# gregorgebhardt/gym-kilobots

Hardware: AMD Instinct MI355X
Metric: kilobot-steps/sec (higher is better)
Workload: dtype f32

## Files before the change

gym_kilobots_amd/csrc/kb_step_kernel.h:

```cpp
#pragma once
#include <type_traits>
#include <utility>

#include "kb_common.h"
#include "kb_objects.h"

namespace kb {

template <int DRIVE_MODE, int LIGHT_TYPE, bool OBJ, int FN = 0, int TIER = 0, bool POLY = true, bool SENSE = true, bool SLEEP = false>
__global__ void __launch_bounds__(TIER == 1 ? 64 : 64 * KB_MAX_WAVES, (TIER == 1 || TIER == 3) ? 2 : ((TIER == 2 || (FN != 0 && !OBJ)) ? KB_COMPACT_WAVES_PER_SIMD : KB_MIN_WAVES_PER_SIMD)) kb_step_kernel(const Params p) {
    constexpr bool WIDE = TIER == 1 || TIER == 3;
    constexpr bool BINS = !OBJ;
    constexpr int KRX = BINS ? KB_KREG_BINS : KREG;
    constexpr bool PAR_DS = FN != 0 && BINS;
    static_assert(!SLEEP || FN == 0 || !OBJ, "the fixed-size instantiations with objects do not carry the sleep state");
    extern __shared__ __align__(16) unsigned char smem[];
    constexpr bool SCOPED = KB_ARGS_SCOPED && FN != 0 && !OBJ;
    using ArgPtr = std::conditional_t<SCOPED, const __attribute__((address_space(4))) Params *, const Params *>;
    ArgPtr ka;
    if constexpr (SCOPED) ka = (ArgPtr)__builtin_amdgcn_kernarg_segment_ptr();
    else ka = &p;
#define KB_REARG() do { if constexpr (SCOPED) { ka = (ArgPtr)__builtin_amdgcn_kernarg_segment_ptr(); asm volatile("" : "+s"(ka)); } } while (0)
    {
        static_assert(sizeof(Params) >= 6 * 64, "the six lines asked for are kernel arguments");
// ... 310 lines not shown
                    float n = sqrtf(lgx * lgx + lgy * lgy);
                    float mx = lgx, my = lgy;
                    if (n > 0.01f) { mx = lgx / n * 0.01f; my = lgy / n * 0.01f; }
                    bvx = mx * WORLD_SCALE; bvy = my * WORLD_SCALE; bww = 0.0f;
                } break;
                default: break;
                }
            }
            if (ka->buf.cmd_vx) { ka->buf.cmd_vx[o + b] = bvx; ka->buf.cmd_vy[o + b] = bvy; ka->buf.cmd_w[o + b] = bww; }
            if (SLEEP) {
                if (drive && slp[q] < 0.0f && (bww * bww > 0.0f || bvx * bvx + bvy * bvy > 0.0f)) slp[q] = 0.0f;
                if (slp[q] < 0.0f) { bvx = 0.0f; bvy = 0.0f; bww = 0.0f; }
                active[b] = 0;
            }
            const float kl = (KB_LAW(q) == KB_DRIVE_SIMPLE_PHOTOTAXIS) ? 1.0f / (1.0f + h * 0.0f) : ka->kl_bot;
            bw[q] = bww * ka->ka_bot;
            int cx = (int)floorf((bx - ka->xmin) * ka->inv_cell);
            int cy = (int)floorf((by - ka->ymin) * ka->inv_cell);
            cx = cx < 0 ? 0 : (cx >= ka->gw ? ka->gw - 1 : cx);
            cy = cy < 0 ? 0 : (cy >= ka->gh ? ka->gh - 1 : cy);
            const int cell = cy * ka->gw + cx;
            if (BINS) {
                sbx[q] = bx; sby[q] = by; svx[q] = bvx * kl; svy[q] = bvy * kl; scell[q] = cx | (cy << 12);
                const int bi = (hashed ? (cell & ka->hmask) : cell) + 1;
                const unsigned old = atomicAdd(reinterpret_cast<unsigned *>(E1) + (bi >> 1), 1u << (16 * (bi & 1)));
                sarr[q] = (int)((old >> (16 * (bi & 1))) & 0xFFFFu);
                if (SENSE && ka->sense_s > 0) reinterpret_cast<unsigned short *>(lAcc)[b] = 0;
            } else {
                vel[b].x = bvx * kl; vel[b].y = bvy * kl;
                parent[b] = b;
                cellOf[b] = (unsigned short)cell;
                nextb[b] = (unsigned short)kb_exch16(head, hix(cell), (unsigned)b);
                if (SENSE && ka->sense_s > 0) newOff[b] = 0;
            }
        }
        if (tid < M) { start[N + tid].x = pos[N + tid].x; start[N + tid].y = pos[N + tid].y; objA0[tid] = objA[tid]; }
        if (tid < M) {
            vel[N + tid].x *= ka->kl_obj; vel[N + tid].y *= ka->kl_obj; objW[tid] *= ka->ka_obj;
            parent[N + tid] = N + tid;
            objCnt[tid] = 0;
            if (SLEEP) active[N + tid] = 0;
        }
        if (OBJ && tid >= M && tid < F) objCnt[tid] = 0;
        if (tid < M_COUNT && tid != M_STATUS) misc[tid] = 0;
        if (SLEEP && tid < 32) misc[M_WAKE + tid] = 0;
        KB_STAMP_PRE(16);
        __syncthreads();
        KB_STAMP(0);
        KB_RETID();
        KB_ABLATE_EXIT(1);
        auto ws_find = [&](int owner, unsigned key16) __attribute__((always_inline)) -> float {
            const int cnt = wsCnt[owner], off = wsOff[owner];
            if (oldInLds) {
                for (int s = 0; s < cnt; ++s)
                    if (oldKey[off + s] == (unsigned short)key16) {
                        const float a_ = oldAcc[off + s];
                        if (SLEEP) oldAcc[off + s] = -1.0f - a_;
                        return a_;
                    }
            } else {
                const unsigned key32 = key16 >= (unsigned)WALL_CODE ? KEY_WALL + (key16 - WALL_CODE)
                                     : (key16 >= (unsigned)OBJ_CODE ? KEY_OBJ + (key16 - OBJ_CODE) : key16);
                for (int s0 = 0; s0 < cnt; s0 += 4) {
                    unsigned k4[4];
#pragma unroll
                    for (int u = 0; u < 4; ++u) {
                        const int idx = off + s0 + u;
                        k4[u] = (s0 + u < cnt && idx < ka->cap) ? ka->buf.ws_key[wo + idx] : 0xFFFFFFFFu;
                    }
#pragma unroll
                    for (int u = 0; u < 4; ++u)
                        if (k4[u] == key32) {
                            const float a_ = ka->buf.ws_acc[wo + off + s0 + u];
                            if (SLEEP) ka->buf.ws_acc[wo + off + s0 + u] = -1.0f - a_;
                            return a_;
                        }
                }
            }
            return -1.0f;
        };
        bool big = false;
        int stageCap = 0, ncon = 0;
        unsigned newTotal = 0;
        if constexpr (BINS) {
            int gw_ = ka->gw, gh_ = ka->gh;
            float invCell_ = ka->inv_cell;
#define KB_GRID_ARGS() do { KB_REARG(); gw_ = ka->gw; gh_ = ka->gh; invCell_ = ka->inv_cell; } while (0)
            {
                const int nchunks = ldsb::bin_entries(ka->nhead) >> 3;
                if (nchunks <= nt) block_scan_bins<true>(E1, nchunks, 1, wsum, tid);
                else block_scan_bins<false>(E1, nchunks, (nchunks + nt - 1) / nt, wsum, tid);
            }
            KB_STAMP_PRE(31);
#pragma unroll
            for (int q = 0; q < BPT; ++q) {
                const int b = tid + q * nt;
                if (b >= N) continue;
                const int cell = SC_CY(scell[q]) * gw_ + SC_CX(scell[q]);
                const int bin = hashed ? (cell & ka->hmask) : cell;
                tmpSort[(int)E1[bin] + sarr[q]] = (unsigned short)b;
            }
            __syncthreads();
            KB_STAMP_PRE(32);
            KB_RETID();
#pragma unroll
            for (int q = 0; q < BPT; ++q) {
                const int b = tid + q * nt;
                if (b >= N) continue;
                const int cell = SC_CY(scell[q]) * gw_ + SC_CX(scell[q]);
                const int bin = hashed ? (cell & ka->hmask) : cell;
                const int s0 = (int)E1[bin], s1 = (int)E1[bin + 1];
                int rank = 0;
                if (s1 - s0 > 1)
                    for (int s_ = s0; s_ < s1; ++s_) rank += ((int)tmpSort[s_] < b) ? 1 : 0;
                const int sl = s0 + rank;
                ms[q] = sl;
                idOf[sl] = (unsigned short)b;
                if (hashed) cellOfSlot[sl] = (unsigned short)cell;
                pos[sl] = make_float2(sbx[q], sby[q]);
                vel[sl] = make_float2(svx[q], svy[q]);
                parent[sl] = (unsigned)sl;
            }
            if (tid < 4) {
                float z_ = 0.0f;
                asm volatile("" : "+v"(z_));
                vel[NB - 5 + tid] = make_float2(z_, z_);
            }
            KB_STAMP_PRE(33);
            KB_GRID_ARGS();
            __syncthreads();
            KB_STAMP(0);
            KB_RETID();
            KB_ABLATE_EXIT(2);
            if (SENSE && ka->sense_s > 0 && drive) {
#pragma unroll 1
                for (int q = 0; q < BPT; ++q) {
                    const int b = tid + q * nt;
                    if (b >= N) continue;
                    const int sl = q == 0 ? ms[0] : ms[BPT - 1];
                    const int sc = q == 0 ? scell[0] : scell[BPT - 1];
                    if (hashed) kb_sense_bins_hashed(pos, E1, cellOfSlot, reinterpret_cast<unsigned *>(lAcc), sl, SC_CX(sc), SC_CY(sc), gw_, gh_, ka->sense_s, ka->sense_r2, ka->hmask);
                    else kb_sense_bins(pos, E1, reinterpret_cast<unsigned *>(lAcc), sl, SC_CX(sc), SC_CY(sc), gw_, gh_, ka->sense_s, ka->sense_r2);
                }
            }
            constexpr int NR = FN ? 3 : 5;
            auto candidate_runs = [&](int sa, int cx, int cy, int (&lo)[NR], int (&hi)[NR], int (&sp)[NR], int (&tc)[5]) __attribute__((always_inline)) {
                const int gw = gw_, gh = gh_;
                const int cell = cy * gw + cx;
                const bool e_ok = cx + 1 < gw, n_ok = cy + 1 < gh, w_ok = cx > 0;
                tc[0] = cell; tc[1] = cell + 1; tc[2] = cell + gw; tc[3] = cell + gw + 1; tc[4] = cell + gw - 1;
                if constexpr (NR == 3) {
                    const int up = cell + gw;
                    const int e1 = (int)E1[cell + 1], e2 = (int)E1[e_ok ? cell + 2 : cell + 1];
                    const int u0 = (int)E1[n_ok ? (w_ok ? up - 1 : up) : 0], u1 = (int)E1[n_ok ? up : 0];
                    const int u2 = (int)E1[n_ok ? up + 1 : 0], u3 = (int)E1[n_ok ? (e_ok ? up + 2 : up + 1) : 0];
                    lo[0] = sa + 1; sp[0] = e1; hi[0] = e2;
                    lo[1] = u1; sp[1] = u2; hi[1] = u3;
                    lo[2] = u0; sp[2] = u1; hi[2] = u1;
                } else {
                    const bool ok[5] = {true, e_ok, n_ok, n_ok && e_ok, n_ok && w_ok};
#pragma unroll
                    for (int k = 0; k < 5; ++k) {
                        const int bin = hashed ? (tc[k] & ka->hmask) : tc[k];
                        const int l_ = ok[k] ? (int)E1[bin] : 0, h_ = ok[k] ? (int)E1[bin + 1] : 0;
                        lo[k] = k == 0 ? sa + 1 : l_; hi[k] = h_; sp[k] = h_;
                    }
// ... 33 lines not shown
                        const float dx = cp[u].x - pa.x, dy = cp[u].y - pa.y;
                        const float dd = dx * dx + dy * dy;
                        bool hit = base + u < tot && !(dd > rr2);
                        if (hashed) {
                            int want = tc[0];
#pragma unroll
                            for (int k = 1; k < 5; ++k) if (ck[u] == k) want = tc[k];
                            hit = hit && cc[u] == want;
                        }
                        if (hit) cb(cs[u], ck[u]);
                    }
                }
            };
            unsigned pl0[BPT], pl1[BPT];
            unsigned snb[BPT], snm[BPT];
#pragma unroll
            for (int q = 0; q < BPT; ++q) {
                const int b = tid + q * nt;
                pl0[q] = 0u; pl1[q] = 0u; snb[q] = 0u; snm[q] = 0u;
                if (b >= N) continue;
                const int sa = ms[q];
                unsigned cnt = 0, nbb = 0, l0 = 0u, l1 = 0u;
                for_partners(sa, SC_CX(scell[q]), SC_CY(scell[q]), [&](int sl, int k) __attribute__((always_inline)) {
                    const unsigned e16 = (unsigned)sl | ((unsigned)k << 12);
                    const unsigned sh = e16 << (16u * (nbb & 1u));
                    l0 |= nbb < 2u ? sh : 0u;
                    l1 |= (nbb >= 2u && nbb < 4u) ? sh : 0u;
                    nbb++;
                    if (((cnt >> (6 * k)) & 63u) == 63u) atomicOr(&misc[M_STATUS], 4u);
                    else cnt += 1u << (6 * k);
                });
                pl0[q] = l0; pl1[q] = l1; snb[q] = nbb;
                unsigned wm = 0u;
                const float ax = pos[sa].x, ay = pos[sa].y;
#pragma unroll
                for (int wl = 0; wl < 4; ++wl) {
                    float dist, nx, ny;
                    wall_geom(*ka, wl, ax, ay, dist, nx, ny);
                    if (dist * dist > rw2) continue;
                    wm |= (1u << wl) | (dist < 0.0f ? 16u << wl : 0u);
                }
                scell[q] |= (int)(wm << 24);
                unsigned mine = nbb + (unsigned)__popc(wm & 15u);
                dirCnt[sa] = cnt;
                if (mine > (unsigned)S) { atomicOr(&misc[M_STATUS], 2u); atomicAdd(&misc[M_XTRA], mine - (unsigned)S); mine = S; }
                wsCntNew[b] = (unsigned char)mine;
                snm[q] = mine;
            }
            KB_STAMP_PRE(17);
            unsigned myOff[BPT];
            {
                static_assert(BPT == 2 && MAX_WAVES <= 8, "two rows of per-wave sums in the 16-word scratch");
                const unsigned inc0 = wave_incl_scan(snm[0]), inc1 = wave_incl_scan(snm[1]);
                if (lane == 63) { wsum[wave] = inc0; wsum[8 + wave] = inc1; }
                KB_GRID_ARGS();
                __syncthreads();
                KB_ABLATE_EXIT(3);
                unsigned b0 = 0, b1 = 0, t0 = 0, t1 = 0;
                for (int w = 0; w < nw; ++w) {
                    const unsigned s0 = wsum[w], s1 = wsum[8 + w];
                    if (w < wave) { b0 += s0; b1 += s1; }
                    t0 += s0; t1 += s1;
                }
                myOff[0] = b0 + inc0 - snm[0]; myOff[1] = t0 + b1 + inc1 - snm[1];
                newTotal = t0 + t1;
            }
            KB_STAMP(1);
            KB_RETID();
            KB_ABLATE_EXIT(4);
            if (SENSE && ka->sense_s > 0 && drive) {
#pragma unroll
                for (int q = 0; q < BPT; ++q) {
                    const int b = tid + q * nt;
                    if (b < N) ka->buf.nbr_count[o + b] = (unsigned)reinterpret_cast<unsigned short *>(lAcc)[ms[q]];
                }
                __syncthreads();
            }
            const unsigned extras = misc[M_XTRA];
            const int capS = FN ? capL_ : min(capL_, ka->cap);
            big = ka->solver_mode >= 3 || newTotal + extras > (unsigned)capS;
            stageCap = big ? ka->cap : capS;
            if (newTotal + extras > (unsigned)stageCap && tid == 0) atomicOr(&misc[M_STATUS], 1u);
            ncon = (int)min(newTotal + extras, (unsigned)stageCap);
            auto stage_pass = [&](unsigned *sPair, unsigned *sInfo) __attribute__((always_inline)) {
#pragma unroll
            for (int q = 0; q < BPT; ++q) {
                const int b = tid + q * nt;
                if (b >= N) continue;
                const int sa = ms[q], cx = SC_CX(scell[q]), cy = SC_CY(scell[q]);
                const unsigned nbb = snb[q];
                const unsigned wm = (unsigned)scell[q] >> 24;
                const unsigned ntot = nbb + (unsigned)__popc(wm & 15u);
                newOff[b] = (unsigned short)myOff[q];
                if (ntot == 0u) continue;
                const unsigned base = myOff[q], nst = snm[q];
                const int cell = cy * gw_ + cx;
                const unsigned common = ((unsigned)(cx & 1) << 12) | ((unsigned)(cy & 1) << 13) | (sa > (int)E1[hashed ? (cell & ka->hmask) : cell] ? 1u << 14 : 0u);
                int curk = -1;
                unsigned jk = 0;
                unsigned wleft = wm & 15u;
                for (unsigned j = 0; j < ntot; ++j) {
                    unsigned pr, inf;
                    if (j < nbb) {
                        unsigned e16;
                        if (j < 4u) e16 = ((j < 2u ? pl0[q] : pl1[q]) >> (16u * (j & 1u))) & 0xFFFFu;
                        else {
                            unsigned idx = 0, f16 = 0;
                            for_partners(sa, cx, cy, [&](int sl, int kk) __attribute__((always_inline)) { if (idx == j) f16 = (unsigned)sl | ((unsigned)kk << 12); idx++; });
                            e16 = f16;
                        }
                        const int k = (int)(e16 >> 12);
                        if (k != curk) { curk = k; jk = 0; } else jk++;
                        if (jk > 255u) { jk = 255u; atomicOr(&misc[M_STATUS], 4u); }
                        pr = (unsigned)sa | ((e16 & 0xFFFu) << 16);
                        inf = (unsigned)k | (jk << 4) | common;
                    } else {
                        const int wl = __builtin_ctz(wleft);
                        wleft &= wleft - 1u;
                        pr = (unsigned)(WALL_CODE + wl) | ((unsigned)sa << 16);
                        inf = (unsigned)(8 + wl) | ((unsigned)__popc(wm & ((1u << wl) - 1u) & 15u) << 4) | (((wm >> (4 + wl)) & 1u) << 15);
                    }
                    const unsigned cid = j < nst ? base + j : newTotal + atomicAdd(&misc[M_XFILL], 1u);
                    if (cid >= (unsigned)stageCap) continue;
                    sPair[cid] = pr;
                    sInfo[cid] = inf;
                }
            }
            };
            if (big) stage_pass(gPair, gInfo); else stage_pass(lPair, lInfo);
            KB_STAMP_PRE(34);
            KB_GRID_ARGS();
            __syncthreads();
            KB_STAMP_PRE(35);
            KB_RETID();
            KB_ABLATE_EXIT(5);
            auto label_pass_bins = [&](unsigned *sPair, unsigned *sInfo, float *sAcc, auto stagedInLds) __attribute__((always_inline)) {
            constexpr bool STAGED_LDS = decltype(stagedInLds)::value;
            for (int c = tid; c < ncon; c += nt) {
                const unsigned pr = sPair[c], raw = sInfo[c];
                const unsigned a = pr & 0xFFFFu, b = pr >> 16;
                unsigned key16, cls, r = (raw >> 4) & 0xFFu;
                float acc;
                if (STAGED_LDS && oldInLds) {
                    const bool wall = a >= (unsigned)WALL_CODE;
                    const unsigned sa_ = wall ? b : a;
                    const unsigned ida = idOf[sa_], idb = idOf[b];
                    unsigned ta = lds_load_relaxed<PAR_DS>(&parent[sa_]), tb = lds_load_relaxed<PAR_DS>(&parent[b]);
                    const int k = wall ? 0 : (int)(raw & 15u);
                    const unsigned keyA = wall ? a : idb;
                    const int cntA = wsCnt[ida], offA = wsOff[ida];
                    const int cntB = wall ? 0 : (int)wsCnt[idb], offB = wsOff[idb];
                    unsigned kA[4], kB[4];
#pragma unroll
                    for (int u = 0; u < 4; ++u) {
                        kA[u] = oldKey[offA + min(u, max(cntA, 1) - 1)];
                        kB[u] = oldKey[offB + min(u, max(cntB, 1) - 1)];
                    }
                    int hitA = -1, hitB = -1;
#pragma unroll
                    for (int u = 3; u >= 0; --u) {
                        if (u < cntA && kA[u] == keyA) hitA = u;
                        if (u < cntB && kB[u] == ida) hitB = u;
                    }
                    if (hitA < 0)
                        for (int s = 4; s < cntA; ++s) if ((unsigned)oldKey[offA + s] == keyA) { hitA = s; break; }
                    if (hitA < 0 && hitB < 0)
                        for (int s = 4; s < cntB; ++s) if ((unsigned)oldKey[offB + s] == ida) { hitB = s; break; }
                    const int ent = hitA >= 0 ? offA + hitA : (hitB >= 0 ? offB + hitB : -1);
                    acc = -1.0f;
                    if (ent >= 0) {
                        acc = oldAcc[ent];
                        if (SLEEP) oldAcc[ent] = -1.0f - acc;
                    }
                    key16 = keyA;
                    if (wall) cls = (unsigned)CLS_WALL | ((raw >> 15) ? 0x80u : 0u);
                    else {
                        const unsigned px = (raw >> 12) & 1u, py = (raw >> 13) & 1u;
                        cls = k == 0 ? (unsigned)CLS_SAME : (k == 1 ? CLS_E + px : (k == 2 ? CLS_N + py : (k == 3 ? CLS_NE + px : CLS_NW + px)));
                        if ((raw >> 14) & 1u) {
                            const float2 pa = pos[a];
                            int cx = (int)floorf((pa.x - ka->xmin) * invCell_);
                            int cy = (int)floorf((pa.y - ka->ymin) * invCell_);
                            cx = cx < 0 ? 0 : (cx >= gw_ ? gw_ - 1 : cx);
                            cy = cy < 0 ? 0 : (cy >= gh_ ? gh_ - 1 : cy);
                            const int cell = cy * gw_ + cx;
                            for (int s_ = (int)E1[hashed ? (cell & ka->hmask) : cell]; s_ < (int)a; ++s_) {
                                if (hashed && (int)cellOfSlot[s_] != cell) continue;
                                r += (dirCnt[s_] >> (6 * k)) & 63u;
                            }
                            if (r > 255u) { r = 255u; atomicOr(&misc[M_STATUS], 4u); }
                        }
                        unsigned ra = a, rb = b;
                        for (;;) {
                            while (ta != ra || tb != rb) {
                                ra = ta; rb = tb;
                                ta = lds_load_relaxed<PAR_DS>(&parent[ra]); tb = lds_load_relaxed<PAR_DS>(&parent[rb]);
                            }
                            if (ra == rb) break;
                            if (ra < rb) { unsigned t = ra; ra = rb; rb = t; }
                            const unsigned seen = atomicCAS(&parent[ra], ra, rb);
                            if (seen == ra) break;
                            ta = seen; tb = rb;
                        }
                    }
                } else if (a >= (unsigned)WALL_CODE) {
                    key16 = a;
                    cls = (unsigned)CLS_WALL | ((raw >> 15) ? 0x80u : 0u);
                    acc = ws_find((int)idOf[b], key16);
                } else {
                    const unsigned ida = idOf[a], idb = idOf[b];
                    const int k = (int)(raw & 15u);
                    const unsigned px = (raw >> 12) & 1u, py = (raw >> 13) & 1u;
                    cls = k == 0 ? (unsigned)CLS_SAME : (k == 1 ? CLS_E + px : (k == 2 ? CLS_N + py : (k == 3 ? CLS_NE + px : CLS_NW + px)));
                    if ((raw >> 14) & 1u) {
                        const float2 pa = pos[a];
                        int cx = (int)floorf((pa.x - ka->xmin) * invCell_);
                        int cy = (int)floorf((pa.y - ka->ymin) * invCell_);
                        cx = cx < 0 ? 0 : (cx >= gw_ ? gw_ - 1 : cx);
                        cy = cy < 0 ? 0 : (cy >= gh_ ? gh_ - 1 : cy);
                        const int cell = cy * gw_ + cx;
                        for (int s_ = (int)E1[hashed ? (cell & ka->hmask) : cell]; s_ < (int)a; ++s_) {
                            if (hashed && (int)cellOfSlot[s_] != cell) continue;
                            r += (dirCnt[s_] >> (6 * k)) & 63u;
                        }
                        if (r > 255u) { r = 255u; atomicOr(&misc[M_STATUS], 4u); }
                    }
                    acc = ws_find((int)ida, idb);
                    if (acc < 0.0f) acc = ws_find((int)idb, ida);
                    key16 = idb;
                    unsigned ra = a, rb = b;
                    for (;;) {
                        while (true) { unsigned t = lds_load_relaxed<PAR_DS>(&parent[ra]); if (t == ra) break; ra = t; }
                        while (true) { unsigned t = lds_load_relaxed<PAR_DS>(&parent[rb]); if (t == rb) break; rb = t; }
                        if (ra == rb) break;
                        if (ra < rb) { unsigned t = ra; ra = rb; rb = t; }
                        if (atomicCAS(&parent[ra], ra, rb) == ra) break;
                    }
                }
                if (acc < 0.0f) acc = 0.0f;
                sInfo[c] = cls | (r << 8) | (key16 << 16);
                sAcc[c] = acc;
            }
            };
            if (big) label_pass_bins(gPair, gInfo, gAcc, std::false_type()); else label_pass_bins(lPair, lInfo, lAcc, std::true_type());
            KB_STAMP_PRE(18);
            __syncthreads();
            KB_STAMP(2);
            KB_RETID();
            KB_ABLATE_EXIT(6);
        } else {
            if (SENSE && ka->sense_s > 0 && drive)
                kb_sense_pass(pos, head, nextb, cellOf, reinterpret_cast<unsigned *>(newOff), N, nt, tid, ka->gw, ka->gh, ka->sense_s, ka->sense_r2, hashed ? ka->hmask : 0);
            if (OBJ && wave == 0) {
                mcTouch = false;
                if (lane < NMC) {
                    owsMine = ka->buf.ows_acc + (size_t)e * (MAXOBJ * KB_OWS_COLS * KB_OWS_WORDS);
                    Arena ar;
                    ar.xmin = ka->xmin; ar.ymin = ka->ymin; ar.xmax = ka->xmax; ar.ymax = ka->ymax;
                    mcTouch = mc_detect(ox, ar, F, lane, owsMine);
                    if (SLEEP && !mcTouch) {
                        int owner_, col_;
                        mc_candidate(F, lane, owner_, col_);
                        if (col_ < 8 && owsMine[(owner_ * KB_OWS_COLS + col_) * KB_OWS_WORDS] >= 0.0f) {
                            const int m1_ = ot_body(objTab + owner_ * OT_WORDS), m2_ = ot_body(objTab + col_ * OT_WORDS);
                            if (m1_ != m2_) {
                                if (objSlp[m1_] < 0.0f) objSlp[m1_] = 0.0f;
                                if (objSlp[m2_] < 0.0f) objSlp[m2_] = 0.0f;
                            }
                        }
                    }
                }
            }

            auto find_pass = [&](unsigned *sPair, unsigned *sInfo, int stageCap_) __attribute__((always_inline)) {
#pragma unroll 1
                for (int a = tid; a < N; a += nt) {
                    const int cell = cellOf[a];
                    const int cx = cell % ka->gw, cy = cell / ka->gw;
                    const float ax = pos[a].x, ay = pos[a].y;
                    unsigned cnt = 0, mine = 0;
                    unsigned hd[5];
                    int tcell[5];
#pragma unroll
                    for (int k = 0; k < 5; ++k) {
                        const int ox = cx + dir_dx(k), oy = cy + dir_dy(k);
                        const bool in = ox >= 0 && ox < ka->gw && oy < ka->gh;
                        tcell[k] = in ? oy * ka->gw + ox : cell;
                        hd[k] = in ? (unsigned)head[hix(tcell[k])] : (unsigned)EMPTY16;
                    }
                    unsigned ckk[5] = {0u, 0u, 0u, 0u, 0u};
                    while (hd[0] != (unsigned)EMPTY16 || hd[1] != (unsigned)EMPTY16 || hd[2] != (unsigned)EMPTY16 ||
                           hd[3] != (unsigned)EMPTY16 || hd[4] != (unsigned)EMPTY16) {
                        float2 pbk[5];
                        unsigned nbk[5];
                        int cbk_[5];
#pragma unroll
                        for (int k = 0; k < 5; ++k) {
                            const unsigned bb = hd[k] != (unsigned)EMPTY16 ? hd[k] : (unsigned)a;
                            pbk[k] = pos[bb]; nbk[k] = nextb[bb];
                            cbk_[k] = hashed ? (int)cellOf[bb] : tcell[k];
                        }
#pragma unroll
                        for (int k = 0; k < 5; ++k) {
                            const unsigned b = hd[k];
                            if (b == (unsigned)EMPTY16) continue;
                            if (!(k == 0 && (int)b <= a) && cbk_[k] == tcell[k]) {
                                const float dx = pbk[k].x - ax, dy = pbk[k].y - ay;
                                const float dd = dx * dx + dy * dy;
                                if (!(dd > rr2)) {
                                    ckk[k]++;
                                    const unsigned c = atomicAdd(&misc[M_NCON], 1u);
                                    if (c < (unsigned)stageCap_) { sPair[c] = (unsigned)a | (b << 16); sInfo[c] = (unsigned)k; }
                                }
                            }
                            hd[k] = nbk[k];
                        }
                    }
#pragma unroll
                    for (int k = 0; k < 5; ++k) {
                        unsigned ck = ckk[k];
                        mine += ck;
                        if (ck > 63u) { ck = 63u; atomicOr(&misc[M_STATUS], 4u); }
                        cnt |= ck << (6 * k);
                    }
#pragma unroll
                    for (int wl = 0; wl < 4; ++wl) {
                        float dist, nx, ny;
// ... 108 lines not shown
                        for (int k2 = 0; k2 < 5; ++k2) nbots += (int)((dc >> (6 * k2)) & 63u);
                        r = 0;
#pragma unroll
                        for (int w2 = 0; w2 < 3; ++w2) {
                            float dist, nx, ny;
                            wall_geom(*ka, w2, ax, ay, dist, nx, ny);
                            if (w2 < wl && !(dist * dist > rw2)) r++;
                        }
                        cls = CLS_WALL | (int)(inf0 & 0x80u);
                        slot = nbots + r;
                        acc = ws_find(a, (unsigned)(WALL_CODE + wl));
                    } else {
                        const int a = pr & 0xFFFF;
                        const unsigned b = pr >> 16;
                        const int cell = cellOf[a];
                        const int cx = cell % ka->gw, cy = cell / ka->gw;
                        const float ax = pos[a].x, ay = pos[a].y;
                        if (k == 0) cls = CLS_SAME;
                        else if (k == 1) cls = CLS_E + (cx & 1);
                        else if (k == 2) cls = CLS_N + (cy & 1);
                        else if (k == 3) cls = CLS_NE + (cx & 1);
                        else cls = CLS_NW + (cx & 1);
                        const unsigned dc = dirCnt[a];
                        int sbase = 0;
                        for (int k2 = 0; k2 < k; ++k2) sbase += (int)((dc >> (6 * k2)) & 63u);
                        int rbase = 0;
                        for (unsigned a2 = head[hix(cell)]; a2 != (unsigned)EMPTY16; a2 = nextb[a2])
                            if ((int)a2 < a && (!hashed || (int)cellOf[a2] == cell)) rbase += (int)((dirCnt[a2] >> (6 * k)) & 63u);
                        int j = 0;
                        if (((dc >> (6 * k)) & 63u) > 1u) {
                            const int oc = (cy + dir_dy(k)) * ka->gw + (cx + dir_dx(k));
                            for (unsigned b2 = head[hix(oc)]; b2 != (unsigned)EMPTY16; b2 = nextb[b2]) {
                                if (b2 >= b || (k == 0 && (int)b2 <= a) || (hashed && (int)cellOf[b2] != oc)) continue;
                                const float2 pb2 = pos[b2];
                                const float ex = pb2.x - ax, ey = pb2.y - ay;
                                if (!(ex * ex + ey * ey > rr2)) j++;
                            }
                        }
                        r = rbase + j;
                        slot = sbase + j;
                        acc = ws_find(a, b);
                        if (acc < 0.0f) acc = ws_find((int)b, (unsigned)a);
                        unsigned ra = a, rb = b;
                        for (;;) {
                            while (true) { unsigned t = lds_load_relaxed<PAR_DS>(&parent[ra]); if (t == ra) break; ra = t; }
                            while (true) { unsigned t = lds_load_relaxed<PAR_DS>(&parent[rb]); if (t == rb) break; rb = t; }
                            if (ra == rb) break;
                            if (ra < rb) { unsigned t = ra; ra = rb; rb = t; }
                            if (atomicCAS(&parent[ra], ra, rb) == ra) break;
                        }
                    }
                    if (acc < 0.0f) acc = 0.0f;
                    if (slot >= S) slot = 255;
                    if (r > 255) { r = 255; atomicOr(&misc[M_STATUS], 4u); }
                    sInfo[c] = (unsigned)cls | ((unsigned)r << 8) | ((unsigned)slot << 16) | fixbits;
                    sAcc[c] = acc;
                }
            };
            if (big) label_pass(gPair, gInfo, gAcc); else label_pass(lPair, lInfo, lAcc);
            KB_STAMP_PRE(18);
            __syncthreads();
            KB_STAMP(2);
            KB_RETID();

        }

        if (SLEEP) {
#pragma unroll
            for (int q = 0; q < BPT; ++q) {
                const int b = tid + q * nt;
                if (b >= N) continue;
                const int cnt = wsCnt[b], off = wsOff[b];
                for (int s_ = 0; s_ < cnt && off + s_ < ka->cap; ++s_) {
                    const float a_ = oldInLds ? oldAcc[off + s_] : ka->buf.ws_acc[wo + off + s_];
                    if (a_ < 0.0f) continue;
                    unsigned key = oldInLds ? (unsigned)oldKey[off + s_] : ka->buf.ws_key[wo + off + s_];
                    if (!oldInLds) key = key >= KEY_OBJ ? OBJ_CODE + (key - KEY_OBJ) : (key >= KEY_WALL ? WALL_CODE + (key - KEY_WALL) : key);
                    if (key >= (unsigned)WALL_CODE) continue;
                    if (slp[q] < 0.0f) slp[q] = 0.0f;
                    if (key >= (unsigned)OBJ_CODE) {
                        if (OBJ) { const int m_ = ot_body(objTab + (key - OBJ_CODE) * OT_WORDS); if (objSlp[m_] < 0.0f) objSlp[m_] = 0.0f; }
                    } else atomicOr(&misc[M_WAKE + (key >> 5)], 1u << (key & 31u));
                }
            }
            __syncthreads();
#pragma unroll
            for (int q = 0; q < BPT; ++q) {
                const int b = tid + q * nt;
                if (b < N && slp[q] < 0.0f && ((misc[M_WAKE + (b >> 5)] >> (b & 31)) & 1u)) slp[q] = 0.0f;
            }
        }
        for (int b = tid; b < N; b += nt) {
            unsigned r = b;
            while (true) { unsigned t = lds_load_relaxed<PAR_DS>(&parent[r]); if (t == r) break; r = t; }
            parent[b] = r;
            islCnt[b] = 0;
            islWave[b] = (unsigned char)((unsigned)b % (unsigned)nsolve);
            if (!BINS) head[hix(cellOf[b])] = EMPTY16;
            if (!SLEEP) active[b] = 1;
            active[NB + b] = 0;
            if (!BINS && SENSE && ka->sense_s > 0 && drive) ka->buf.nbr_count[o + b] = (unsigned)newOff[b];
        }
        if (tid < 64) bkStart[tid] = 0;
        if (tid < 32) bkFill[tid] = 0;
        if (tid < M) {
            const int b = N + tid;
            unsigned r = b;
            while (true) { unsigned t = lds_load_relaxed<PAR_DS>(&parent[r]); if (t == r) break; r = t; }
            parent[b] = r;
            islCnt[b] = 0;
            islWave[b] = (unsigned char)((unsigned)b % (unsigned)nw);
            if (!SLEEP) active[b] = 1;
            active[NB + b] = 0;
        }
        if (SLEEP && !BINS) {
#pragma unroll
            for (int q = 0; q < BPT; ++q) {
                const int b = tid + q * nt;
                if (b < N && !(slp[q] < 0.0f)) active[parent[b]] = 1;
            }
            if (tid < M && !(objSlp[tid] < 0.0f)) active[parent[N + tid]] = 1;
        }
        if (BINS) __syncthreads();
        else newTotal = block_scan_u8(wsCntNew, newOff, NP, wsum, tid);
        if (SLEEP && BINS) {
#pragma unroll
            for (int q = 0; q < BPT; ++q) {
                const int b = tid + q * nt;
                if (b < N && !(slp[q] < 0.0f)) active[parent[ms[q]]] = 1;
            }
        }
        const bool newInLds = BINS ? !big : newTotal <= (unsigned)capL_;
        if (OBJ && wave == 0) {
            unsigned root = 0;
            const bool on = lane < NMC && mcTouch;
            if (on) { root = parent[mci(ox, MC_B, lane)]; mci_set(ox, MC_ISL, lane, (int)root); }
        }
        KB_STAMP(14);
        KB_RETID();
        KB_ABLATE_EXIT(7);
        const bool wcntDead = BINS && nw > 1 && ka->solver_mode == 0;
        auto census = [&](const unsigned *sPair) __attribute__((always_inline)) {
            for (int c = tid; c < ncon; c += nt) {
                const unsigned root = parent[sPair[c] >> 16];
                const unsigned n = atomicAdd(&islCnt[root], 1u) + 1u;
                if (n > (unsigned)GIANT_ISLAND) atomicMax(&misc[M_MAXISL], n);
                if (!wcntDead) atomicAdd(&misc[M_WCNT + islWave[root]], 1u);
            }
        };
        if (big) census(gPair); else census(lPair);
        __syncthreads();
        unsigned maxw = 0;
        for (int w = 0; w < nw; ++w) maxw = max(maxw, misc[M_WCNT + w]);
        bool coopForced = misc[M_MAXISL] > (unsigned)GIANT_ISLAND || ka->solver_mode == 2 || ka->solver_mode == 4;
        bool coop = coopForced || nw == 1;
        if (!coop && !big && ka->solver_mode == 0) {
            unsigned *szSum = bkStart, *szPre = bkStart + 32, *szFill = bkFill, *szTab = bkFill + 32;
            static_assert(MAX_WAVES <= 32 && lds::nbk(2) >= 32 + MAX_WAVES, "szTab: a word per wave behind the 32 class counters");
            for (int b = tid; b < N + M; b += nt) {
                if (parent[b] != (unsigned)b) continue;
                const unsigned cnt_ = islCnt[b];
                if (cnt_ != 0) atomicAdd(&szSum[32u - min(cnt_, 32u)], cnt_);
            }
            __syncthreads();
            if (wave == 0) {
                const unsigned v_ = lane < 32 ? szSum[lane] : 0u;
                const unsigned incl = wave_incl_scan(v_);
                if (lane < 32) szPre[lane] = incl - v_;
                if constexpr (BINS) {
                    const unsigned excl = incl - v_;
                    const unsigned s_ = 32u - min(lane, 31u);
                    const unsigned mg_ = (unsigned)(65536.5f * __builtin_amdgcn_rcpf((float)s_)) + 1u;
                    const unsigned total = (unsigned)__builtin_amdgcn_readlane((int)incl, 31);
                    bool even = __builtin_amdgcn_readfirstlane((int)v_) != 0;
                    bool two = false;
                    unsigned pos = 0, first = lane == 0u ? 0u : total;
                    if (!even) {
#pragma unroll
                        for (unsigned w = 0; w < (unsigned)nsolve; ++w) {
                            if (pos >= total) break;
                            const unsigned s = 32u - (unsigned)__builtin_ctzll(__ballot(incl > pos));
                            two = two || total - pos + s > ((unsigned)nsolve - 1u - w) * (129u - s) + 65u;
                            const unsigned end = pos + (two ? 128u : 64u);
                            const unsigned long long m_ = __ballot(incl > end);
                            unsigned nxt = total;
                            if (m_ != 0ull) {
                                const int q = __builtin_ctzll(m_);
                                const unsigned start = max(pos, (unsigned)__builtin_amdgcn_readlane((int)excl, q));
                                nxt = start + (((end - start) * (unsigned)__builtin_amdgcn_readlane((int)mg_, q)) >> 16) * (32u - (unsigned)q);
                            }
                            first = lane == w + 1u ? nxt : first;
                            pos = nxt;
                        }
                        even = pos < total;
                    }
                    const unsigned mine = even ? 0u : (unsigned)__shfl_down((int)first, 1) - first;
                    if (even) first = lane * max(((unsigned)ncon + (unsigned)nsolve - 1u) / (unsigned)nsolve, 1u);
                    if (lane >= (unsigned)nsolve) first = 0xFFFFFFFFu;
                    if (lane < MAX_WAVES) szTab[lane] = lane == 0u ? (even ? 1u : 0u) : first;
                    if (lane < nw) misc[M_WCNT + lane] = mine;
                } else if (lane < nw) misc[M_WCNT + lane] = 0;
            }
            __syncthreads();
            if constexpr (BINS) {
                unsigned st_[MAX_WAVES];
#pragma unroll
                for (int k = 0; k < MAX_WAVES; ++k) st_[k] = szTab[k];
                const bool even = st_[0] != 0u;
                for (int b = tid; b < N + M; b += nt) {
                    if (parent[b] != (unsigned)b) continue;
                    const unsigned cnt_ = islCnt[b];
                    if (cnt_ == 0) continue;
                    const unsigned q_ = 32u - min(cnt_, 32u);
                    const unsigned at = szPre[q_] + atomicAdd(&szFill[q_], cnt_);
                    unsigned w_ = 0;
#pragma unroll
                    for (int k = 1; k < MAX_WAVES; ++k) w_ += at >= st_[k] ? 1u : 0u;
                    islWave[b] = (unsigned char)w_;
                    if (even) atomicAdd(&misc[M_WCNT + w_], cnt_);
                }
            } else {
                unsigned chunk = 60u;
                if ((unsigned)ncon > 60u * (unsigned)(nw - 1) + 124u) chunk = ((unsigned)ncon - 124u + (unsigned)nw - 2u) / (unsigned)(nw - 1);
                for (int b = tid; b < N + M; b += nt) {
                    if (parent[b] != (unsigned)b) continue;
                    const unsigned cnt_ = islCnt[b];
                    if (cnt_ == 0) continue;
                    const unsigned q_ = 32u - min(cnt_, 32u);
                    const unsigned at = szPre[q_] + atomicAdd(&szFill[q_], cnt_);
                    const unsigned w_ = min(at / max(chunk, 1u), (unsigned)nsolve - 1u);
                    islWave[b] = (unsigned char)w_;
                    atomicAdd(&misc[M_WCNT + w_], cnt_);
                }
            }
            __syncthreads();
            maxw = 0;
            for (int w = 0; w < nw; ++w) maxw = max(maxw, misc[M_WCNT + w]);
        }
        bool reg = !coopForced && !big && maxw <= 64u * KRX && ka->solver_mode == 0;
        if (!coop && !big && maxw > 64u * KRX && ka->solver_mode == 0) {
            unsigned short *bigList = bkList;
            __syncthreads();
            if (tid < nw) misc[M_WCNT + tid] = 0;
            if (tid == 0) misc[M_TOTAL] = 0;
            __syncthreads();
            for (int b = tid; b < N + M; b += nt) {
                if (parent[b] != (unsigned)b) continue;
                const unsigned cnt_ = islCnt[b];
                if (cnt_ == 0) continue;
                unsigned slot_ = 64u;
                if (cnt_ >= (unsigned)BIG_ISLAND) slot_ = atomicAdd(&misc[M_TOTAL], 1u);
                if (slot_ < 64u) bigList[slot_] = (unsigned short)b;
                else atomicAdd(&misc[M_WCNT + islWave[b]], cnt_);
            }
            __syncthreads();
            if (wave == 0) {
                const int nb = (int)min(misc[M_TOTAL], 64u);
                const unsigned root = lane < nb ? (unsigned)bigList[lane] : 0u;
                const unsigned size = lane < nb ? islCnt[root] : 0u;
                int rank = 0;
                for (int j = 0; j < nb; ++j) {
                    const unsigned sj = __shfl(size, j), rj = __shfl(root, j);
                    if (sj > size || (sj == size && rj < root)) rank++;
                }
                unsigned load = lane < nsolve ? misc[M_WCNT + lane] : 0u;
                int myWave = 0;
                for (int r = 0; r < nb; ++r) {
                    const int src = __builtin_ctzll(__ballot(lane < nb && rank == r));
                    const unsigned sz = __shfl(size, src);
                    unsigned key = lane < nsolve ? ((load << 4) | (unsigned)lane) : 0xFFFFFFFFu;
                    for (int d = 8; d >= 1; d >>= 1) key = min(key, __shfl_xor(key, d));
                    const int wmin = (int)(__shfl(key, 0) & 15u);
                    if (lane == wmin) load += sz;
                    if (lane == src) myWave = wmin;
                }
                if (lane < nb) islWave[root] = (unsigned char)myWave;
                if (lane < nsolve) misc[M_WCNT + lane] = load;
            }
            __syncthreads();
            maxw = 0;
            for (int w = 0; w < nw; ++w) maxw = max(maxw, misc[M_WCNT + w]);
            reg = maxw <= 64u * KRX;
        }
        if (BINS && nw > 1 && !reg && ka->solver_mode == 0) { coopForced = true; coop = true; }
        if (OBJ && wave == 0) {
            const bool on = lane < NMC && mcTouch && (!SLEEP || active[mci(ox, MC_ISL, lane)] != 0);
            const unsigned w_ = on ? (unsigned)islWave[mci(ox, MC_ISL, lane)] : 0u;
            for (int w = 0; w < nw; ++w) {
                const unsigned long long mk = __ballot(on && (int)w_ == w);
                if (lane == 0) mcMask[w] = mk;
            }
            const unsigned long long all = __ballot(on);
            if (lane == 0) mcMask[nw] = all;
        }
        auto mc_warm_pass = [&](unsigned long long mask, bool leader) __attribute__((always_inline)) {
            if (leader) for (unsigned long long m_ = mask; m_; m_ &= m_ - 1) mc_warm_start(ox, __builtin_ctzll(m_));
        };
        auto mc_velocity_pass = [&](unsigned long long mask, bool leader) __attribute__((always_inline)) {
            if (leader) for (unsigned long long m_ = mask; m_; m_ &= m_ - 1) mc_solve_velocity(ox, __builtin_ctzll(m_));
        };
        auto mc_position_pass = [&](unsigned long long mask, bool leader, const unsigned char *act, unsigned char *nxt, bool lastIt) __attribute__((always_inline)) -> bool {
            bool viol = false;
            if (leader)
                for (unsigned long long m_ = mask; m_; m_ &= m_ - 1) {
                    const int t = __builtin_ctzll(m_);
                    const int isl = mci(ox, MC_ISL, t);
                    if (!act[isl]) continue;
                    const float minSep = mc_solve_position(ox, t, B2_BAUMGARTE);
                    if (minSep < -3.0f * B2_LINEAR_SLOP) { nxt[isl] = 1; viol = true; if (SLEEP && lastIt) islWave[isl] = 3; }
                }
            return viol;
        };
        auto mc_clear_flags = [&](unsigned long long mask, bool leader, unsigned char *act) __attribute__((always_inline)) {
            if (leader) for (unsigned long long m_ = mask; m_; m_ &= m_ - 1) act[mci(ox, MC_ISL, __builtin_ctzll(m_))] = 0;
        };
        auto mc_store = [&]() __attribute__((always_inline)) {
            if (OBJ && wave == 0 && lane < NMC) {
                int owner, col;
                mc_candidate(F, lane, owner, col);
                float *dst = owsMine + (owner * KB_OWS_COLS + col) * KB_OWS_WORDS;
                float o[KB_OWS_WORDS] = {-1.0f, -1.0f, -1.0f, -1.0f, -1.0f, -1.0f};
                if (mcTouch) {
                    const int cnt = (mci(ox, MC_TYPE, lane) >> 2) & 3, ids = mci(ox, MC_ID, lane);
                    o[0] = (float)(ids & 255); o[1] = mcf(ox, MC_NI0, lane); o[2] = mcf(ox, MC_TI0, lane);
                    if (cnt == 2) { o[3] = (float)((ids >> 8) & 255); o[4] = mcf(ox, MC_NI1, lane); o[5] = mcf(ox, MC_TI1, lane); }
                }
#pragma unroll
                for (int k = 0; k < KB_OWS_WORDS; ++k) dst[k] = o[k];
            }
        };
        auto bucket_sort = [&](const unsigned *sPair, const unsigned *sInfo, unsigned short *cbk,
                               unsigned short *order) __attribute__((always_inline)) {
            const int W = coop ? 1 : nw;
            for (int b = tid; b < N + M; b += nt) islCnt[b] = 0;
            for (int k = tid; k < W * BK_PER_WAVE; k += nt) { bkStart[k] = 0; bkFill[k] = 0; }
            for (int k = tid; k < W * NUM_CLS; k += nt) bkMaxRank[k] = 0;
            if (tid == 0) bkStart[W * BK_PER_WAVE] = 0;
            __syncthreads();
            for (int c = tid; c < ncon; c += nt) {
                const unsigned root = parent[sPair[c] >> 16];
                if (SLEEP && !active[root]) { cbk[c] = EMPTY16; continue; }
                const int w = coop ? 0 : (int)islWave[root];
                const unsigned inf = sInfo[c];
                const int cls = inf & 0x7F, r = (inf >> 8) & 0xFF;
                const int bk = (w * NUM_CLS + cls) * RK + (r < RK - 1 ? r : RK - 1);
                cbk[c] = (unsigned short)bk;
                atomicAdd(&bkStart[bk], 1u);
                if (r >= RK - 1) atomicMax(&bkMaxRank[w * NUM_CLS + cls], (unsigned)r);
            }
            __syncthreads();
            if (wave == 0) {
                const int nb = W * BK_PER_WAVE;
                const int chunk = (nb + 63) / 64;
                const int s0 = lane * chunk, e0 = min(nb, s0 + chunk);
                unsigned sum = 0;
                for (int i = s0; i < e0; ++i) sum += bkStart[i];
                const unsigned incl = wave_incl_scan(sum);
                unsigned run = incl - sum;
                for (int i = s0; i < e0; ++i) { unsigned v = bkStart[i]; bkStart[i] = run; run += v; }
                if (lane == 63) bkStart[nb] = incl;
            }
            __syncthreads();
            for (int c = tid; c < ncon; c += nt) {
                const int bk = cbk[c];
                if (SLEEP && bk == (int)EMPTY16) continue;
                order[bkStart[bk] + atomicAdd(&bkFill[bk], 1u)] = (unsigned short)c;
            }
            if (wave < W) {
                const int base = wave * BK_PER_WAVE;
                const bool ne = lane < BK_PER_WAVE && bkStart[base + lane + 1] > bkStart[base + lane];
                const unsigned long long m = __ballot(ne);
                if (ne) bkList[base + __popcll(m & ((1ull << lane) - 1ull))] = (unsigned short)(base + lane);
                if (lane == 0) nList[wave] = (unsigned char)__popcll(m);
            }
            __syncthreads();
        };
        SolveArgs ca;
        if (reg) {
            for (int b = tid; b < N + M; b += nt) islCnt[b] = 0;
            if (tid < nw * NUM_CLS) bkMaxRank[tid] = 0;
            if constexpr (BINS) {
                if (tid < 32) intMark[tid] = 0;
                if (wave_s == 0) {
                    const unsigned v_ = lane < nw ? misc[M_WCNT + lane] : 0u;
                    const unsigned incl = wave_incl_scan(v_);
                    if (lane < nw) misc[M_WFILL + lane] = incl - v_;
                }
                __syncthreads();
                for (int c = tid; c < ncon; c += nt) {
                    const unsigned pr = lPair[c], a = pr & 0xFFFFu, b = pr >> 16;
                    const unsigned root = parent[b];
                    const unsigned w = islWave[root];
                    lOrder[atomicAdd(&misc[M_WFILL + w], 1u)] = (unsigned short)c;
                    if (!SLEEP || active[root] != 0) {
                        atomicOr(&intMark[b & 31u], 1u << (b >> 5));
                        if (a < (unsigned)WALL_CODE) atomicOr(&intMark[a & 31u], 1u << (a >> 5));
                    }
                }
            } else {
                for (int c = tid; c < ncon; c += nt) {
                    const unsigned w = islWave[parent[lPair[c] >> 16]];
                    unsigned base = 0;
                    for (unsigned w2 = 0; w2 < w; ++w2) base += misc[M_WCNT + w2];
                    lOrder[base + atomicAdd(&misc[M_WFILL + w], 1u)] = (unsigned short)c;
                }
            }
            if (BINS) { KB_REARG(); ca = solve_args(*ka); }
            __syncthreads();
        } else if (big) bucket_sort(gPair, gInfo, gCbk, gOrder);
        else bucket_sort(lPair, lInfo, lCbk, lOrder);
        KB_STAMP(3);
        KB_RETID();
        if (!(BINS && reg)) ca = solve_args(*ka);
        KB_ABLATE_EXIT(8);

        const bool coopLevels = BINS && coopForced && nw > 1;
        if constexpr (BINS) {
            if (reg) {
#include "kb_regsolve_bins.inc"
            } else if (coopLevels) {
#include "kb_coopsolve_bins.inc"
            }
        }
        if (BINS && (reg || coopLevels)) {
        } else if (reg) {
            unsigned mybase = 0;
            for (int w = 0; w < wave; ++w) mybase += misc[M_WCNT + w];
            const unsigned mycnt = misc[M_WCNT + wave];
            int ra[KREG], rb[KREG], rkey[KREG], rrank[KREG], rslot[KREG], risl[KREG], rc[KREG], rdepth[KREG];
            float racc[KREG], rnx[KREG], rny[KREG], rima[KREG], rimb[KREG], rra[KREG], rrb[KREG], rnm[KREG];
            bool rvalid[KREG], rflip[KREG];
            bool rpoly[KREG];
            float rrAx[KREG], rrAy[KREG], rlnx[KREG], rlny[KREG], rlpx[KREG], rlpy[KREG];
            unsigned mlo = 0, mhi = 0;
            const float nm_bb = ca.nm_bb, nm_wb = ca.nm_wb;
#define R_IMA(j) (OBJ ? rima[j] : (ra[j] < WALL_CODE ? ca.im_bot : 0.0f))
#define R_IMB(j) (OBJ ? rimb[j] : ca.im_bot)
#define R_RA(j) (OBJ ? rra[j] : (ra[j] < WALL_CODE ? ca.r_bot : B2_POLYGON_RADIUS))
#define R_RB(j) (OBJ ? rrb[j] : ca.r_bot)
#define R_NM(j) (OBJ ? rnm[j] : (ra[j] < WALL_CODE ? nm_bb : nm_wb))
#pragma unroll
            for (int j = 0; j < KREG; ++j) {
                const unsigned idx = lane + 64u * j;
                rvalid[j] = idx < mycnt;
                ra[j] = 0; rb[j] = 0; rkey[j] = 0; rrank[j] = 0; rc[j] = 0; rdepth[j] = 0;
                if (rvalid[j]) {
                    const int c = lOrder[mybase + idx];
                    const unsigned pr = lPair[c], inf = lInfo[c];
                    const int cls = inf & 0x7F, r = (inf >> 8) & 0xFF;
                    rc[j] = c; ra[j] = pr & 0xFFFF; rb[j] = pr >> 16; rrank[j] = r;
                    const int key = cls * RK + (r < RK - 1 ? r : RK - 1);
                    if (SLEEP && !active[parent[rb[j]]]) {
                        rkey[j] = -1;
                    } else {
                        rkey[j] = key;
                        if (key < 32) mlo |= 1u << key; else mhi |= 1u << (key - 32);
                        if (r >= RK - 1) atomicMax(&bkMaxRank[wave * NUM_CLS + cls], (unsigned)r);
                    }
                }
            }
            mlo = wave_or(mlo); mhi = wave_or(mhi);
            const unsigned long long keymask = ((unsigned long long)mhi << 32) | mlo;
            wave_sync();
#ifdef KB_PROFILE
            if (tid == 0) { atomicAdd(&KB_PROF(8), (unsigned)__popcll(keymask)); atomicAdd(&KB_PROF(11), 1u); }
#endif

#define KB_REG_KEY_ROUNDS(...)                                                                      \
            for (unsigned long long m_ = keymask; m_; m_ &= m_ - 1) {                               \
                const int key_ = __builtin_ctzll(m_);                                               \
                if ((key_ % RK) < RK - 1) {                                                         \
// ... 970 lines not shown
```

Before: 18.02 billion.

## Derive island counts from per-body contact counts during flatten, skipping census pass

When contacts are owned per body (bins path, multi-wave, no extras), island sizes are accumulated during the parent-flatten pass from per-body new contact counts minus stale direction counts, instead of a separate census over contacts. The class-size sums are then computed once up front, and for the uneven split the wave fill offsets are written directly so a later scan and barrier are skipped. This removes a pass over contacts and a block-wide barrier, at the cost of extra LDS atomics and more complex bookkeeping that must stay consistent with the earlier counts.

```diff
diff --git a/gym_kilobots_amd/csrc/kb_step_kernel.h b/gym_kilobots_amd/csrc/kb_step_kernel.h
--- a/gym_kilobots_amd/csrc/kb_step_kernel.h
+++ b/gym_kilobots_amd/csrc/kb_step_kernel.h
@@ -416,6 +416,10 @@
         bool big = false;
         int stageCap = 0, ncon = 0;
         unsigned newTotal = 0;
+        bool ownedCnt = false;
+        unsigned dirStale[BPT];
+#pragma unroll
+        for (int q = 0; q < BPT; ++q) dirStale[q] = 0u;
         if constexpr (BINS) {
             int gw_ = ka->gw, gh_ = ka->gh;
             float invCell_ = ka->inv_cell;
@@ -615,6 +619,7 @@
             stageCap = big ? ka->cap : capS;
             if (newTotal + extras > (unsigned)stageCap && tid == 0) atomicOr(&misc[M_STATUS], 1u);
             ncon = (int)min(newTotal + extras, (unsigned)stageCap);
+            ownedCnt = nw > 1 && ka->solver_mode == 0 && !big && extras == 0u;
             auto stage_pass = [&](unsigned *sPair, unsigned *sInfo) __attribute__((always_inline)) {
 #pragma unroll
             for (int q = 0; q < BPT; ++q) {
@@ -776,6 +781,13 @@
             }
             };
             if (big) label_pass_bins(gPair, gInfo, gAcc, std::false_type()); else label_pass_bins(lPair, lInfo, lAcc, std::true_type());
+            if (!SLEEP && ownedCnt) {
+#pragma unroll
+                for (int q = 0; q < BPT; ++q) {
+                    const int b = tid + q * nt;
+                    if (b < N) dirStale[q] = dirCnt[b];
+                }
+            }
             KB_STAMP_PRE(18);
             __syncthreads();
             KB_STAMP(2);
@@ -1050,6 +1062,7 @@
                         if (OBJ) { const int m_ = ot_body(objTab + (key - OBJ_CODE) * OT_WORDS); if (objSlp[m_] < 0.0f) objSlp[m_] = 0.0f; }
                     } else atomicOr(&misc[M_WAKE + (key >> 5)], 1u << (key & 31u));
                 }
+                if (BINS && ownedCnt) islCnt[b] = 0;
             }
             __syncthreads();
 #pragma unroll
@@ -1058,16 +1071,30 @@
                 if (b < N && slp[q] < 0.0f && ((misc[M_WAKE + (b >> 5)] >> (b & 31)) & 1u)) slp[q] = 0.0f;
             }
         }
-        for (int b = tid; b < N; b += nt) {
+        auto flatten_slot = [&](int b, unsigned stale) __attribute__((always_inline)) {
+            unsigned own = 0;
+            if (BINS && ownedCnt) own = wsCntNew[idOf[b]];
             unsigned r = b;
             while (true) { unsigned t = lds_load_relaxed<PAR_DS>(&parent[r]); if (t == r) break; r = t; }
             parent[b] = r;
-            islCnt[b] = 0;
+            if (BINS && ownedCnt) {
+                if (stale != 0u) atomicSub(&islCnt[b], stale);
+                if (own != 0u) atomicAdd(&islCnt[r], own);
+            } else islCnt[b] = 0;
             islWave[b] = (unsigned char)((unsigned)b % (unsigned)nsolve);
             if (!BINS) head[hix(cellOf[b])] = EMPTY16;
             if (!SLEEP) active[b] = 1;
             active[NB + b] = 0;
             if (!BINS && SENSE && ka->sense_s > 0 && drive) ka->buf.nbr_count[o + b] = (unsigned)newOff[b];
+        };
+        if constexpr (BINS) {
+#pragma unroll
+            for (int q = 0; q < BPT; ++q) {
+                const int b = tid + q * nt;
+                if (b < N) flatten_slot(b, dirStale[q]);
+            }
+        } else {
+            for (int b = tid; b < N; b += nt) flatten_slot(b, 0u);
         }
         if (tid < 64) bkStart[tid] = 0;
         if (tid < 32) bkFill[tid] = 0;
@@ -1116,21 +1143,30 @@
                 if (!wcntDead) atomicAdd(&misc[M_WCNT + islWave[root]], 1u);
             }
         };
-        if (big) census(gPair); else census(lPair);
+        unsigned *szSum = bkStart, *szPre = bkStart + 32, *szFill = bkFill, *szTab = bkFill + 32;
+        auto class_sums = [&](bool giant) __attribute__((always_inline)) {
+            for (int b = tid; b < N + M; b += nt) {
+                if (parent[b] != (unsigned)b) continue;
+                const unsigned cnt_ = islCnt[b];
+                if (cnt_ != 0) atomicAdd(&szSum[32u - min(cnt_, 32u)], cnt_);
+                if (giant && cnt_ > (unsigned)GIANT_ISLAND) atomicMax(&misc[M_MAXISL], cnt_);
+            }
+        };
+        if (BINS && ownedCnt) class_sums(true);
+        else if (big) census(gPair);
+        else census(lPair);
         __syncthreads();
         unsigned maxw = 0;
         for (int w = 0; w < nw; ++w) maxw = max(maxw, misc[M_WCNT + w]);
         bool coopForced = misc[M_MAXISL] > (unsigned)GIANT_ISLAND || ka->solver_mode == 2 || ka->solver_mode == 4;
         bool coop = coopForced || nw == 1;
+        bool evenSplit = true;
         if (!coop && !big && ka->solver_mode == 0) {
-            unsigned *szSum = bkStart, *szPre = bkStart + 32, *szFill = bkFill, *szTab = bkFill + 32;
             static_assert(MAX_WAVES <= 32 && lds::nbk(2) >= 32 + MAX_WAVES, "szTab: a word per wave behind the 32 class counters");
-            for (int b = tid; b < N + M; b += nt) {
-                if (parent[b] != (unsigned)b) continue;
-                const unsigned cnt_ = islCnt[b];
-                if (cnt_ != 0) atomicAdd(&szSum[32u - min(cnt_, 32u)], cnt_);
-            }
-            __syncthreads();
+            if (!(BINS && ownedCnt)) {
+                class_sums(false);
+                __syncthreads();
+            }
             if (wave == 0) {
                 const unsigned v_ = lane < 32 ? szSum[lane] : 0u;
                 const unsigned incl = wave_incl_scan(v_);
@@ -1163,6 +1199,7 @@
                         even = pos < total;
                     }
                     const unsigned mine = even ? 0u : (unsigned)__shfl_down((int)first, 1) - first;
+                    if (!even && lane < nw) misc[M_WFILL + lane] = first;
                     if (even) first = lane * max(((unsigned)ncon + (unsigned)nsolve - 1u) / (unsigned)nsolve, 1u);
                     if (lane >= (unsigned)nsolve) first = 0xFFFFFFFFu;
                     if (lane < MAX_WAVES) szTab[lane] = lane == 0u ? (even ? 1u : 0u) : first;
@@ -1175,6 +1212,8 @@
 #pragma unroll
                 for (int k = 0; k < MAX_WAVES; ++k) st_[k] = szTab[k];
                 const bool even = st_[0] != 0u;
+                evenSplit = even;
+                if (!even && tid < 32) intMark[tid] = 0;
                 for (int b = tid; b < N + M; b += nt) {
                     if (parent[b] != (unsigned)b) continue;
                     const unsigned cnt_ = islCnt[b];
@@ -1208,6 +1247,7 @@
         bool reg = !coopForced && !big && maxw <= 64u * KRX && ka->solver_mode == 0;
         if (!coop && !big && maxw > 64u * KRX && ka->solver_mode == 0) {
             unsigned short *bigList = bkList;
+            evenSplit = true;
             __syncthreads();
             if (tid < nw) misc[M_WCNT + tid] = 0;
             if (tid == 0) misc[M_TOTAL] = 0;
@@ -1348,13 +1388,15 @@
             for (int b = tid; b < N + M; b += nt) islCnt[b] = 0;
             if (tid < nw * NUM_CLS) bkMaxRank[tid] = 0;
             if constexpr (BINS) {
-                if (tid < 32) intMark[tid] = 0;
-                if (wave_s == 0) {
-                    const unsigned v_ = lane < nw ? misc[M_WCNT + lane] : 0u;
-                    const unsigned incl = wave_incl_scan(v_);
-                    if (lane < nw) misc[M_WFILL + lane] = incl - v_;
-                }
-                __syncthreads();
+                if (evenSplit) {
+                    if (tid < 32) intMark[tid] = 0;
+                    if (wave_s == 0) {
+                        const unsigned v_ = lane < nw ? misc[M_WCNT + lane] : 0u;
+                        const unsigned incl = wave_incl_scan(v_);
+                        if (lane < nw) misc[M_WFILL + lane] = incl - v_;
+                    }
+                    __syncthreads();
+                }
                 for (int c = tid; c < ncon; c += nt) {
                     const unsigned pr = lPair[c], a = pr & 0xFFFFu, b = pr >> 16;
                     const unsigned root = parent[b];
```

Measured after the change: 18.03 billion, median of 5. No clear change (+0.0%).
